# Arcadia-Science/arcadia-microscopy-tools

Hardware: AMD Instinct MI355X
Metric: fields-of-view/sec (4x2048^2 uint16) end-to-end segment+props (higher is better)
Workload: dtype f64; 1 GPU; configs[2]: synthetic 4-channel 2048x2048 uint16 FOVs, DAPI Gaussian+Otsu+open/close+EDT+peak markers+watershed nuclei (SEEDED relief, seeds_first: marker pixels spread first in raster order, cannot tie; SURVEY A.8's plain -EDT relief with exact ties is reported under sublines.a8_exact) + clear_border/relabel + morphology and 4-channel intensity regionprops; mode=weak scaling, 192 FOVs per GPU per step, streams_per_gpu=4, fovs_per_launch=48, max_cells_per_fov=2048, distinct_fovs_per_gpu=8, resident_in_hbm=True

## Files before the change

arcadia_microscopy_tools_amd/_thresholds.py:

```python
from __future__ import annotations

import numpy as np
from scipy import ndimage as ndi


def counts_centers_u16(hist65536: np.ndarray):
    nz = np.flatnonzero(hist65536)
    lo, hi = int(nz[0]), int(nz[-1])
    return hist65536[lo:hi + 1].astype(np.int64), np.arange(lo, hi + 1)


def counts_centers_f64(hist: np.ndarray, vmin: float, vmax: float):
    edges = np.linspace(vmin, vmax, len(hist) + 1)
    return hist.astype(np.int64), (edges[:-1] + edges[1:]) / 2.0


def otsu(counts, bin_centers):
    counts = counts.astype(float)
    if len(bin_centers) == 1:
        return bin_centers[0]
    w_lo = np.cumsum(counts)
    w_hi = np.cumsum(counts[::-1])[::-1]
    weighted = counts * bin_centers
    m_lo = np.cumsum(weighted) / w_lo
# ... 82 lines not shown
        raise RuntimeError("Maximum iteration reached for histogram smoothing")
    k = np.argmin(smooth[maxima[0]:maxima[1] + 1])
    return bin_centers[maxima[0] + k]


def mean_from_hist(counts, values):
    return float(np.sum(counts * values)) / float(np.sum(counts))


def li_from_hist(counts, values, tolerance=None, initial_guess=None, wrap_dtype=None):
    values = values.astype(np.int64)
    counts = np.asarray(counts)
    image_min = int(values[0])
    v = values - image_min
    if wrap_dtype is not None and np.dtype(wrap_dtype).kind == "i" and int(v[-1]) > int(np.iinfo(wrap_dtype).max):
        half = int(np.iinfo(wrap_dtype).max) + 1
        v = (v + half) % (2 * half) - half
        order = np.argsort(v, kind="stable")
        v, counts = v[order], counts[order]
    present = v[counts > 0]
    if present.size == 1:
        return values[0]
    tolerance = tolerance or np.min(np.diff(present)) / 2
    total_sum = np.sum(counts * v)
    total_cnt = np.sum(counts)
    t_next = total_sum / total_cnt if initial_guess is None else initial_guess - image_min
    t_curr = -2 * tolerance
    csum = np.cumsum(counts * v)
    ccnt = np.cumsum(counts)
    with np.errstate(invalid="ignore", divide="ignore"):
        while abs(t_next - t_curr) > tolerance:
            t_curr = t_next
            k = int(np.searchsorted(v, t_curr, side="right")) - 1
            s_le = csum[k] if k >= 0 else 0
            c_le = ccnt[k] if k >= 0 else 0
            mean_back = np.float64(s_le) / np.float64(c_le)
            mean_fore = np.float64(total_sum - s_le) / np.float64(total_cnt - c_le)
            t_next = (mean_back - mean_fore) / (np.log(mean_back) - np.log(mean_fore))
    return t_next + image_min


def prefix_rule(v: np.ndarray, vmin: float, vmax: float, nbins: int = 256):
    v = np.ascontiguousarray(v, dtype=np.float64)
    if (v < 0).any():
        raise ValueError("the prefix order holds for non-negative samples only")
    hi32 = v.view(np.uint64) >> np.uint64(32) << np.uint64(32)
    vlo, vhi = hi32.view(np.float64), (hi32 | np.uint64(0xFFFFFFFF)).view(np.float64)
    edges = np.linspace(vmin, vmax, nbins + 1)
    bins = np.clip(np.searchsorted(edges, vlo, side="right") - 1, 0, nbins - 1)
    centres = (edges[:-1] + edges[1:]) / 2.0
    above = vlo > centres[bins]
    undecided = ((bins < nbins - 1) & (vhi >= edges[bins + 1])) | (~above & (vhi > centres[bins]))
    return bins, above, undecided
```

arcadia_microscopy_tools_amd/csrc/amt_props.hip:

```cpp
#include "amt_internal.h"

#include <vector>

typedef unsigned long long u64;

enum { A_N = 0, A_SY, A_SX, A_SYY, A_SXX, A_SXY, A_C1, A_C2, A_C3, A_NACC };

__global__ void __launch_bounds__(256) rp_init_kernel(u64* __restrict__ acc, int* __restrict__ bbox, size_t nlab) {
    for (size_t i = (size_t)blockIdx.x * 256 + threadIdx.x; i < nlab; i += (size_t)gridDim.x * 256) {
        for (int k = 0; k < A_NACC; ++k) acc[i * A_NACC + k] = 0;
        bbox[i * 4 + 0] = 0x7fffffff;
        bbox[i * 4 + 1] = 0x7fffffff;
        bbox[i * 4 + 2] = -1;
        bbox[i * 4 + 3] = -1;
    }
}

__device__ __forceinline__ u64 sum_sq_upto(u64 m) { return m * (m + 1) * (2 * m + 1) / 6; }

__device__ __forceinline__ double diff_of_products(u64 a, u64 b, u64 c, u64 d) {
    u64 lo1 = a * b, hi1 = __umul64hi(a, b);
    u64 lo2 = c * d, hi2 = __umul64hi(c, d);
    bool neg = (hi1 < hi2) || (hi1 == hi2 && lo1 < lo2);
    u64 hi, lo;
    if (!neg) {
        lo = lo1 - lo2;
        hi = hi1 - hi2 - (lo1 < lo2 ? 1 : 0);
    } else {
        lo = lo2 - lo1;
        hi = hi2 - hi1 - (lo2 < lo1 ? 1 : 0);
    }
    double v = (double)hi * 18446744073709551616.0 + (double)lo;
    return neg ? -v : v;
}

__global__ void __launch_bounds__(256) rp_bbox_kernel(const int* __restrict__ labels, int* __restrict__ bbox, int H,
                                                      int W, int max_label) {
    const int lane = threadIdx.x & 63;
    const int x = blockIdx.x * 64 + lane;
    const int yb = (blockIdx.y * 4 + (threadIdx.x >> 6)) * 8;
    if (yb >= H) return;
    const size_t n = (size_t)H * W;
    const int plane = blockIdx.z;
    int labs[8];
#pragma unroll
    for (int k = 0; k < 8; ++k) {
        const int y = yb + k;
        int v = 0;
        if (x < W && y < H) v = labels[(size_t)plane * n + (size_t)y * W + x];
        labs[k] = (v < 0 || v > max_label) ? 0 : v;
    }
#pragma unroll
    for (int k = 0; k < 8; ++k) {
        const int lab = labs[k];
        const int left = __shfl_up(lab, 1);
        const bool head = (lane == 0) || (left != lab);
        const u64 heads = __ballot(head);
        if (lab != 0 && head) {
            const u64 later = heads & ~((2ull << lane) - 1ull);
            const int end_lane = later ? (__ffsll((long long)later) - 2) : 63;
            int* B = bbox + ((size_t)plane * max_label + (lab - 1)) * 4;
            atomicMin(&B[0], yb + k);
            atomicMin(&B[1], x);
            atomicMax(&B[2], yb + k);
            atomicMax(&B[3], x + (end_lane - lane));
        }
    }
}

__device__ __forceinline__ u64 wave_sum_u64(u64 v) {
#pragma unroll
    for (int off = 32; off >= 1; off >>= 1) v += __shfl_xor(v, off);
    return v;
}
__device__ __forceinline__ unsigned wave_min_u32(unsigned v) {
#pragma unroll
    for (int off = 32; off >= 1; off >>= 1) {
        unsigned t = __shfl_xor(v, off);
        v = t < v ? t : v;
    }
    return v;
}
__device__ __forceinline__ unsigned wave_max_u32(unsigned v) {
#pragma unroll
    for (int off = 32; off >= 1; off >>= 1) {
        unsigned t = __shfl_xor(v, off);
        v = t > v ? t : v;
    }
    return v;
}

constexpr int RP_MAXC = 4;
__global__ void __launch_bounds__(64) rp_label_kernel(const int* __restrict__ labels, const int* __restrict__ bbox,
                                                      const int* __restrict__ hoff, const int* __restrict__ htot,
                                                      int2* __restrict__ rows, size_t cap, u64* __restrict__ acc,
                                                      const uint16_t* __restrict__ inten, int C, int c0, int nc,
                                                      double* __restrict__ itable, int H, int W, int max_label,
                                                      int want_morph) {
    const int plane = blockIdx.y;
    const int l = blockIdx.x;
    const int lane = threadIdx.x;
    const size_t li = (size_t)plane * max_label + l;
    const int y0 = bbox[li * 4 + 0], x0 = bbox[li * 4 + 1], y1 = bbox[li * 4 + 2], x1 = bbox[li * 4 + 3];
    if (y1 < y0) {
        if (itable && lane < 4 * nc) itable[(li * C + c0) * 4 + lane] = 0.0;
        return;
    }
    const size_t n = (size_t)H * W;
    const int* L = labels + (size_t)plane * n;
    const uint16_t* I = inten ? inten + ((size_t)plane * C + c0) * n : nullptr;
    const int want = l + 1;
    const bool rows_ok = want_morph && (size_t)htot[plane] <= cap;
    int2* myrows = rows + (size_t)plane * cap + (size_t)hoff[li];
    u64 cnt = 0, sy = 0, sx = 0, syy = 0, sxx = 0, sxy = 0;
    u64 s[RP_MAXC], q[RP_MAXC];
    unsigned mn[RP_MAXC], mx[RP_MAXC];
#pragma unroll
    for (int c = 0; c < RP_MAXC; ++c) {
        s[c] = 0;
        q[c] = 0;
        mn[c] = 0xffffffffu;
        mx[c] = 0;
    }
    constexpr int RPS = 3;
    for (int yb = y0; yb <= y1; yb += RPS) {
        int rmin[RPS], rmax[RPS];
#pragma unroll
        for (int j = 0; j < RPS; ++j) {
            rmin[j] = 0x7fffffff;
            rmax[j] = -1;
        }
        for (int xb = x0; xb <= x1; xb += 64) {
            const int x = xb + lane;
            unsigned bcnt = 0, bsy = 0;
            const int xc = x <= x1 ? x : x1;
            int lv[RPS];
#pragma unroll
            for (int j = 0; j < RPS; ++j) {
                const int yc = yb + j <= y1 ? yb + j : y1;
                lv[j] = L[(size_t)yc * W + xc];
            }
            unsigned iv[RPS][RP_MAXC];
            if (I) {
#pragma unroll
                for (int j = 0; j < RPS; ++j) {
                    const int yc = yb + j <= y1 ? yb + j : y1;
#pragma unroll
                    for (int c = 0; c < RP_MAXC; ++c) iv[j][c] = I[(size_t)(c < nc ? c : 0) * n + (size_t)yc * W + xc];
                }
            }
#pragma unroll
            for (int j = 0; j < RPS; ++j)
                if (x > x1 || yb + j > y1) lv[j] = 0;
#pragma unroll
            for (int j = 0; j < RPS; ++j) {
                const int y = yb + j;
                const bool m = lv[j] == want;
                if (m) {
                    bcnt += 1u;
                    bsy += (unsigned)y;
                    syy += (u64)(unsigned)y * (unsigned)y;
                    if (I) {
#pragma unroll
                        for (int c = 0; c < RP_MAXC; ++c)
                            if (c < nc) {
                                const unsigned v = iv[j][c];
                                s[c] += v;
                                q[c] += (u64)v * v;
                                mn[c] = v < mn[c] ? v : mn[c];
                                mx[c] = v > mx[c] ? v : mx[c];
                            }
                    }
                }
                const u64 bal = __ballot(m);
                if (bal) {
                    const int first = xb + __ffsll((long long)bal) - 1;
                    const int last = xb + 63 - __clzll((long long)bal);
                    rmin[j] = first < rmin[j] ? first : rmin[j];
                    rmax[j] = last > rmax[j] ? last : rmax[j];
                }
            }
            cnt += bcnt;
            sy += bsy;
            sx += (u64)(unsigned)x * bcnt;
            sxx += (u64)(unsigned)x * (unsigned)x * bcnt;
            sxy += (u64)(unsigned)x * bsy;
        }
        if (rows_ok && lane == 0) {
#pragma unroll
            for (int j = 0; j < RPS; ++j)
                if (yb + j <= y1) myrows[yb + j - y0] = make_int2(rmin[j], rmax[j]);
        }
    }
    cnt = wave_sum_u64(cnt);
    if (want_morph) {
        sy = wave_sum_u64(sy);
        sx = wave_sum_u64(sx);
        syy = wave_sum_u64(syy);
        sxx = wave_sum_u64(sxx);
        sxy = wave_sum_u64(sxy);
        if (lane == 0) {
            u64* A = acc + li * A_NACC;
            A[A_N] = cnt;
            A[A_SY] = sy;
            A[A_SX] = sx;
            A[A_SYY] = syy;
            A[A_SXX] = sxx;
            A[A_SXY] = sxy;
        }
    }
    if (itable) {
#pragma unroll
        for (int c = 0; c < RP_MAXC; ++c)
            if (c < nc) {
                const u64 S = wave_sum_u64(s[c]), Q = wave_sum_u64(q[c]);
                const unsigned lo = wave_min_u32(mn[c]), hi = wave_max_u32(mx[c]);
                if (lane == 0) {
                    double* t = itable + (li * C + c0 + c) * 4;
                    if (cnt == 0) {
                        t[0] = t[1] = t[2] = t[3] = 0.0;
                    } else {
                        const double dn = (double)cnt;
                        t[0] = (double)S / dn;
                        t[1] = (double)hi;
                        t[2] = (double)lo;
                        const double nv = diff_of_products(cnt, Q, S, S);
                        const double var = nv / (dn * dn);
                        t[3] = sqrt(var < 0.0 ? 0.0 : var);
                    }
                }
            }
    }
}

constexpr int PR_ROWS = 64, PR_IN = 60, PR_BATCH = 17, PR_NBATCH = (PR_ROWS + 4) / PR_BATCH;
static_assert(PR_BATCH * PR_NBATCH == PR_ROWS + 4, "row batches must tile the strip");

__global__ void __launch_bounds__(256) rp_perimeter_rows_kernel(const int* __restrict__ labels, u64* __restrict__ acc,
                                                                int H, int W, int max_label, int* __restrict__ bbox) {
    const int lane = threadIdx.x & 63;
    const int strip = blockIdx.x * 4 + (threadIdx.x >> 6);
    if (strip * PR_IN >= W) return;
    const int plane = blockIdx.z;
    const size_t n = (size_t)H * W;
    const int* L = labels + (size_t)plane * n;
    const int x = strip * PR_IN - 2 + lane;
    const int y0 = blockIdx.y * PR_ROWS;
    const bool xin = x >= 0 && x < W;
    const bool inner = xin && lane >= 2 && lane < 2 + PR_IN;
    const unsigned ml = (unsigned)max_label;
    u64* accp = acc + (size_t)plane * max_label * A_NACC;
    int* bbp = bbox ? bbox + (size_t)plane * max_label * 4 : nullptr;

    const int xc = x < 0 ? 0 : (x < W ? x : W - 1);
    auto load_row = [&](int y) -> int {
        const int yc = y < 0 ? 0 : (y < H ? y : H - 1);
        return L[(size_t)yc * W + xc];
    };
    int cur[PR_BATCH], nxt[PR_BATCH];
#pragma unroll
    for (int j = 0; j < PR_BATCH; ++j) cur[j] = load_row(y0 - 2 + j);
    int v1 = 0, v1l = 0, v1r = 0, v2 = 0, v2l = 0, v2r = 0;
    int wA = 0, wAl = 0, wAr = 0, wB = 0, wBl = 0, wBr = 0;
    for (int b = 0; b < PR_NBATCH; ++b) {
        if (b + 1 < PR_NBATCH) {
#pragma unroll
            for (int j = 0; j < PR_BATCH; ++j) nxt[j] = load_row(y0 - 2 + (b + 1) * PR_BATCH + j);
        }
#pragma unroll
        for (int j = 0; j < PR_BATCH; ++j) {
            const int r = y0 - 2 + b * PR_BATCH + j;
            int v0 = cur[j];
            v0 = (xin && r >= 0 && r < H && (unsigned)(v0 - 1) < ml) ? v0 : 0;
            if (__ballot((v0 | v1 | v2 | wB) != 0) == 0ull) continue;
            const int v0l = amt_lane_left(v0), v0r = amt_lane_right(v0);
            const bool b1 = v1 != 0 && (v2 != v1 || v0 != v1 || v1l != v1 || v1r != v1);
            const int w1 = b1 ? (v1 | (int)0x80000000) : v1;
            const int w1l = amt_lane_left(w1), w1r = amt_lane_right(w1);
            const int yb = r - 1;
            if (bbp && yb >= y0 && yb < y0 + PR_ROWS) {
                const bool live = inner && v1 != 0, head = live && v1l != v1;
                const bool q0 = head && v2 != v1, q2 = head && v0 != v1, q1 = head && v2l != v1 && v0l != v1;
                const bool q3 = live && v1r != v1 && v2r != v1 && v0r != v1;
                if (__ballot(q0 || q1 || q2 || q3)) {
                    int* B = bbp + (size_t)(v1 - 1) * 4;
                    if (q0) atomicMin(&B[0], yb);
                    if (q2) atomicMax(&B[2], yb);
                    if (q1) atomicMin(&B[1], x);
                    if (q3) atomicMax(&B[3], x);
                }
            }
            const int yo = r - 2;
            if (inner && wA < 0 && yo >= y0 && yo < y0 + PR_ROWS) {
                const int key = wA;
                const int code = 1 + 2 * ((wB == key) + (w1 == key) + (wAl == key) + (wAr == key)) +
                                 10 * ((wBl == key) + (wBr == key) + (w1l == key) + (w1r == key));
                constexpr unsigned long long M1 = (1ull << 5) | (1ull << 7) | (1ull << 15) | (1ull << 17) | (1ull << 25) | (1ull << 27);
                constexpr unsigned long long M2 = (1ull << 21) | (1ull << 33), M3 = (1ull << 13) | (1ull << 23);
                const int cls = ((M1 >> code) & 1ull) ? A_C1 : ((M2 >> code) & 1ull) ? A_C2 : ((M3 >> code) & 1ull) ? A_C3 : -1;
                if (cls >= 0) atomicAdd(&accp[(size_t)((key & 0x7fffffff) - 1) * A_NACC + cls], 1ull);
            }
            wB = wA, wBl = wAl, wBr = wAr;
            wA = w1, wAl = w1l, wAr = w1r;
            v2 = v1, v2l = v1l, v2r = v1r;
            v1 = v0, v1l = v0l, v1r = v0r;
        }
#pragma unroll
        for (int j = 0; j < PR_BATCH; ++j) cur[j] = nxt[j];
    }
}

__global__ void __launch_bounds__(256) rp_heights_kernel(const int* __restrict__ bbox, int* __restrict__ hoff,
                                                         int max_label) {
    const int plane = blockIdx.y;
    for (int l = blockIdx.x * 256 + threadIdx.x; l < max_label; l += gridDim.x * 256) {
        const int* B = bbox + ((size_t)plane * max_label + l) * 4;
        hoff[(size_t)plane * max_label + l] = B[2] >= B[0] ? B[2] - B[0] + 1 : 0;
    }
}

constexpr int HULL_HMAX = 48, HULL_WMAX = 250;

__device__ __forceinline__ long long floor_div(long long a, long long b) {
    long long q = a / b;
    return (a % b != 0 && a < 0) ? q - 1 : q;
}
__device__ __forceinline__ long long ceil_div(long long a, long long b) {
    long long q = a / b;
    return (a % b != 0 && a > 0) ? q + 1 : q;
}

template <bool CROWS>
__global__ void __launch_bounds__(64) rp_hull_kernel(const int* __restrict__ bbox, const int* __restrict__ hoff,
                                                     const int* __restrict__ htot, const int2* __restrict__ rows,
                                                     int2* __restrict__ chainL, int2* __restrict__ chainR, size_t cap,
                                                     double* __restrict__ table, int max_label, int skip_h,
                                                     int2* __restrict__ crows) {
    const int plane = blockIdx.y;
    const int l = blockIdx.x * 64 + threadIdx.x;
    if (l >= max_label) return;
    const size_t li = (size_t)plane * max_label + l;
    double* trow = CROWS ? nullptr : table + li * AMT_RP_NCOLS;
    const int miny = bbox[li * 4 + 0], maxy = bbox[li * 4 + 2];
    if (maxy < miny) {
        if (!CROWS && skip_h == 0) trow[AMT_RP_AREA_CONVEX] = 0.0;
        return;
    }
    const int h = maxy - miny + 1;
    if (h <= skip_h && bbox[li * 4 + 3] - bbox[li * 4 + 1] + 1 <= HULL_WMAX) return;
    const size_t off = (size_t)hoff[li];
    if ((size_t)htot[plane] > cap || off + (size_t)h > cap) {
        if (!CROWS) trow[AMT_RP_AREA_CONVEX] = __longlong_as_double(0x7ff8000000000000ll);
        return;
    }
    const int2* r = rows + (size_t)plane * cap + off;
    int2* CL = chainL + (size_t)plane * 3 * cap + 3 * off;
    int2* CR = chainR + (size_t)plane * 3 * cap + 3 * off;
    int nl = 0, nr = 0;
    for (int Y = 2 * miny - 1; Y <= 2 * maxy + 1; ++Y) {
        int mn = 0x7fffffff, mx = -0x7fffffff;
        if (Y & 1) {
// ... 208 lines not shown
        const double n2 = dn * dn;
        const double a = Nxx / n2;
        const double c = Nyy / n2;
        const double b = -Nxy / n2;
        const double tr = (a + c) * 0.5;
        const double hd = (a - c) * 0.5;
        const double rad = sqrt(hd * hd + b * b);
        double l1 = tr + rad, l2 = tr - rad;
        l1 = l1 < 0.0 ? 0.0 : l1;
        l2 = l2 < 0.0 ? 0.0 : l2;
        t[AMT_RP_AXIS_MAJOR] = 4.0 * sqrt(l1);
        t[AMT_RP_AXIS_MINOR] = 4.0 * sqrt(l2);
        t[AMT_RP_ECCENTRICITY] = l1 == 0.0 ? 0.0 : sqrt(1.0 - l2 / l1);
        double orient;
        if (Nxx == Nyy) {
            orient = (Nxy > 0.0) ? -0.78539816339744828 : 0.78539816339744828;
        } else {
            orient = 0.5 * atan2(-2.0 * b, c - a);
        }
        t[AMT_RP_ORIENTATION] = orient;
    }
}

__global__ void __launch_bounds__(256) rp_solidity_kernel(double* __restrict__ table, size_t nlab) {
    for (size_t i = (size_t)blockIdx.x * 256 + threadIdx.x; i < nlab; i += (size_t)gridDim.x * 256) {
        double* t = table + i * AMT_RP_NCOLS;
        t[AMT_RP_SOLIDITY] = t[AMT_RP_AREA] > 0.0 ? t[AMT_RP_AREA] / t[AMT_RP_AREA_CONVEX] : 0.0;
    }
}

extern "C" int amt_regionprops(amt_ctx* ctx, const int32_t* labels, const uint16_t* intensity, int C, double* table_dev,
                               double* itable_dev, int nplanes, int H, int W, int max_label) {
    AMT_REQUIRE(labels && (table_dev || itable_dev) && nplanes >= 0 && H > 0 && W > 0 && max_label >= 0,
                "regionprops: bad arguments");
    AMT_REQUIRE(!intensity == !itable_dev && (!itable_dev || C >= 1),
                "regionprops: the intensity planes (C >= 1) and the intensity table go together");
    AMT_TRY(amt_set_device(ctx));
    const bool want_morph = table_dev != nullptr;
    if (nplanes == 0 || max_label == 0) return AMT_OK;
    const size_t n = (size_t)H * W;
    const size_t nlab = (size_t)nplanes * max_label;
    const size_t cap = want_morph ? n : 1;
    amt_scratch s(ctx);
    amt_buf<u64> acc(s, nlab * A_NACC);
    amt_buf<int> bbox(s, nlab * 4);
    amt_buf<int> hoff(s, nlab);
    amt_buf<int> htot(s, nplanes);
    amt_buf<int2> rows(s, (size_t)nplanes * cap);
    amt_buf<int2> chainL(s, (size_t)nplanes * 3 * cap);
    amt_buf<int2> chainR(s, (size_t)nplanes * 3 * cap);
    AMT_TRY(s.commit());
    hipLaunchKernelGGL(rp_init_kernel, dim3(amt_grid_for(nlab, 256, 1024)), dim3(256), 0, ctx->stream, acc, bbox, nlab);
    AMT_LAUNCH_CHECK();
    if (want_morph) {
        const int nstrips = (W + PR_IN - 1) / PR_IN;
        dim3 gper((nstrips + 3) / 4, (H + PR_ROWS - 1) / PR_ROWS, nplanes);
        hipLaunchKernelGGL(rp_perimeter_rows_kernel, gper, dim3(256), 0, ctx->stream, labels, acc, H, W, max_label, bbox);
    } else {
        hipLaunchKernelGGL(rp_bbox_kernel, dim3((W + 63) / 64, (H + 31) / 32, nplanes), dim3(256), 0, ctx->stream,
                           labels, bbox, H, W, max_label);
    }
    AMT_LAUNCH_CHECK();
    hipLaunchKernelGGL(rp_heights_kernel, dim3(amt_grid_for(max_label, 256, 256), nplanes), dim3(256), 0, ctx->stream,
                       bbox, hoff, max_label);
    AMT_LAUNCH_CHECK();
    AMT_TRY(amt_scan_excl(ctx, hoff, max_label, (size_t)max_label, htot, nplanes));
    const int groups = intensity ? (C + RP_MAXC - 1) / RP_MAXC : 1;
    for (int g = 0; g < groups; ++g) {
        const int c0 = g * RP_MAXC;
        const int nc = intensity ? ((C - c0) < RP_MAXC ? (C - c0) : RP_MAXC) : 0;
        hipLaunchKernelGGL(rp_label_kernel, dim3(max_label, nplanes), dim3(64), 0, ctx->stream, labels, bbox, hoff, htot,
                           rows, cap, acc, intensity, C, c0, nc, intensity ? itable_dev : (double*)nullptr, H, W,
                           max_label, (want_morph && g == 0) ? 1 : 0);
        AMT_LAUNCH_CHECK();
    }
    if (want_morph) {
        hipLaunchKernelGGL(rp_final_kernel, dim3(amt_grid_for(nlab, 256, 1024)), dim3(256), 0, ctx->stream, acc, bbox,
                           table_dev, nlab);
        AMT_LAUNCH_CHECK();
        const int skip_h = HULL_HMAX;
        hipLaunchKernelGGL(rp_hull_lds_kernel<false>, dim3((max_label + 31) / 32, nplanes), dim3(64), 0, ctx->stream, bbox,
                           hoff, htot, rows, cap, table_dev, max_label, (int2*)nullptr);
        AMT_LAUNCH_CHECK();
        hipLaunchKernelGGL(rp_hull_kernel<false>, dim3((max_label + 63) / 64, nplanes), dim3(64), 0, ctx->stream, bbox,
                           hoff, htot, rows, chainL, chainR, cap, table_dev, max_label, skip_h, (int2*)nullptr);
        AMT_LAUNCH_CHECK();
        hipLaunchKernelGGL(rp_solidity_kernel, dim3(amt_grid_for(nlab, 256, 1024)), dim3(256), 0, ctx->stream,
                           table_dev, nlab);
        AMT_LAUNCH_CHECK();
    }
    return AMT_OK;
}

__global__ void __launch_bounds__(256) bbox_init_kernel(int* __restrict__ bbox, size_t nlab) {
    for (size_t i = (size_t)blockIdx.x * 256 + threadIdx.x; i < nlab; i += (size_t)gridDim.x * 256) {
        bbox[i * 4 + 0] = 0x7fffffff;
        bbox[i * 4 + 1] = 0x7fffffff;
        bbox[i * 4 + 2] = -1;
        bbox[i * 4 + 3] = -1;
    }
}

__global__ void __launch_bounds__(64) rp_intensity_f64_kernel(const int* __restrict__ labels, const int* __restrict__ bbox,
                                                              const double* __restrict__ inten, int C,
                                                              double* __restrict__ itable, int H, int W, int max_label) {
    const int plane = blockIdx.y, l = blockIdx.x, lane = threadIdx.x;
    const size_t li = (size_t)plane * max_label + l;
    const int y0 = bbox[li * 4 + 0], x0 = bbox[li * 4 + 1], y1 = bbox[li * 4 + 2], x1 = bbox[li * 4 + 3];
    double* out = itable + li * (size_t)C * 4;
    if (y1 < y0) {
        for (int i = lane; i < C * 4; i += 64) out[i] = 0.0;
        return;
    }
    const size_t n = (size_t)H * W;
    const int* lab = labels + (size_t)plane * n;
    auto wsum = [&](double v) {
#pragma unroll
        for (int o = 32; o > 0; o >>= 1) v += __shfl_xor(v, o);
        return v;
    };
    for (int c = 0; c < C; ++c) {
        const double* img = inten + ((size_t)plane * C + c) * n;
        double s = 0.0, cnt = 0.0, mn = __longlong_as_double(0x7ff0000000000000ll), mx = -mn;
        for (int y = y0; y <= y1; ++y)
            for (int x = x0 + lane; x <= x1; x += 64)
                if (lab[(size_t)y * W + x] == l + 1) {
                    const double v = img[(size_t)y * W + x];
                    s += v;
                    cnt += 1.0;
                    mn = v < mn ? v : mn;
                    mx = v > mx ? v : mx;
                }
        s = wsum(s);
        cnt = wsum(cnt);
#pragma unroll
        for (int o = 32; o > 0; o >>= 1) {
            const double a = __shfl_xor(mn, o), b = __shfl_xor(mx, o);
            mn = a < mn ? a : mn;
            mx = b > mx ? b : mx;
        }
        const double mean = s / cnt;
        double q = 0.0;
        for (int y = y0; y <= y1; ++y)
            for (int x = x0 + lane; x <= x1; x += 64)
                if (lab[(size_t)y * W + x] == l + 1) {
                    const double d = img[(size_t)y * W + x] - mean;
                    q += d * d;
                }
        q = wsum(q);
        if (lane == 0) {
            out[c * 4 + 0] = mean;
            out[c * 4 + 1] = mx;
            out[c * 4 + 2] = mn;
            out[c * 4 + 3] = sqrt(q / cnt);
        }
    }
}

extern "C" int amt_regionprops_intensity_f64(amt_ctx* ctx, const int32_t* labels, const double* intensity, int C,
                                             double* table_dev, int nplanes, int H, int W, int max_label) {
    AMT_TRY(amt_set_device(ctx));
    AMT_REQUIRE(labels && intensity && table_dev && nplanes >= 0 && H > 0 && W > 0 && max_label >= 0 && C >= 1,
                "regionprops_intensity_f64: bad arguments");
    if (nplanes == 0 || max_label == 0) return AMT_OK;
    const size_t nlab = (size_t)nplanes * max_label;
    amt_scratch s(ctx);
    amt_buf<int> bbox(s, nlab * 4);
    AMT_TRY(s.commit());
    hipLaunchKernelGGL(bbox_init_kernel, dim3(amt_grid_for(nlab, 256, 1024)), dim3(256), 0, ctx->stream, bbox, nlab);
    AMT_LAUNCH_CHECK();
    hipLaunchKernelGGL(rp_bbox_kernel, dim3((W + 63) / 64, (H + 31) / 32, nplanes), dim3(256), 0, ctx->stream, labels, bbox,
                       H, W, max_label);
    AMT_LAUNCH_CHECK();
    hipLaunchKernelGGL(rp_intensity_f64_kernel, dim3(max_label, nplanes), dim3(64), 0, ctx->stream, labels, bbox, intensity, C,
                       table_dev, H, W, max_label);
    AMT_LAUNCH_CHECK();
    return AMT_OK;
}

extern "C" int amt_label_bboxes(amt_ctx* ctx, const int32_t* labels, int32_t* bbox_dev, int nplanes, int H, int W,
                                int max_label) {
    AMT_TRY(amt_set_device(ctx));
    AMT_REQUIRE(labels && bbox_dev && nplanes >= 0 && H > 0 && W > 0 && max_label >= 1, "label_bboxes: bad arguments");
    if (nplanes == 0) return AMT_OK;
    const size_t nlab = (size_t)nplanes * max_label;
    hipLaunchKernelGGL(bbox_init_kernel, dim3(amt_grid_for(nlab, 256, 1024)), dim3(256), 0, ctx->stream, bbox_dev, nlab);
    AMT_LAUNCH_CHECK();
    hipLaunchKernelGGL(rp_bbox_kernel, dim3((W + 63) / 64, (H + 31) / 32, nplanes), dim3(256), 0, ctx->stream, labels,
                       bbox_dev, H, W, max_label);
    AMT_LAUNCH_CHECK();
    return AMT_OK;
}


__global__ void __launch_bounds__(64) rpx_quad_kernel(const int* __restrict__ labels, const int* __restrict__ bbox,
                                                      double* __restrict__ table, int H, int W, int max_label,
                                                      int want_euler, int want_crofton) {
    __shared__ unsigned hist[16];
    const int plane = blockIdx.y, l = blockIdx.x, lane = threadIdx.x;
    const size_t li = (size_t)plane * max_label + l;
    if (lane < 16) hist[lane] = 0;
    __syncthreads();
    const int y0 = bbox[li * 4 + 0], x0 = bbox[li * 4 + 1], y1 = bbox[li * 4 + 2], x1 = bbox[li * 4 + 3];
    const int* L = labels + (size_t)plane * H * W;
    const int want = l + 1;
    if (y1 >= y0) {
        for (int xb = x0; xb <= x1 + 1; xb += 64) {
            const int x = xb + lane;
            const bool col = x <= x1 + 1;
            unsigned up = 0, upl = 0;
            for (int y = y0; y <= y1 + 1; ++y) {
                unsigned c = 0, cl = 0;
                if (col && y <= y1) {
                    if (x <= x1) c = L[(size_t)y * W + x] == want;
                    if (x - 1 >= x0) cl = L[(size_t)y * W + x - 1] == want;
                }
                const unsigned code = c | (up << 1) | (cl << 2) | (upl << 3);
                if (col && code != 0 && code != 15) atomicAdd(&hist[code], 1u);
                up = c;
                upl = cl;
            }
        }
    }
    __syncthreads();
    if (lane == 0) {
        double* t = table + li * AMT_RPX_NCOLS;
        long long h[16];
        for (int k = 0; k < 16; ++k) h[k] = hist[k];
        if (want_euler) t[AMT_RPX_COL_EULER_NUMBER] = (double)(h[8] - h[6] - h[14]);
        if (want_crofton) {
            const double pi = 3.141592653589793, s2 = sqrt(2.0);
            const double coefs[16] = {0, pi / 4 * (1 + 1 / s2), pi / (4 * s2), pi / (2 * s2), 0, pi / 4 * (1 + 1 / s2),
                                      0, pi / (4 * s2), pi / 4, pi / 2, pi / (4 * s2), pi / (4 * s2), pi / 4, pi / 2, 0, 0};
            double p = 0.0;
            for (int k = 0; k < 16; ++k) p += coefs[k] * (double)h[k];
            t[AMT_RPX_COL_PERIMETER_CROFTON] = y1 >= y0 ? p : 0.0;
        }
    }
}

constexpr int HOLE_SMALL = 64;
__device__ __forceinline__ u64 row_fill(u64 r, u64 b) {
// ... 284 lines not shown
                }
#pragma unroll
        for (int o = 32; o >= 1; o >>= 1) {
            s += __shfl_xor(s, o);
            sy += __shfl_xor(sy, o);
            sx += __shfl_xor(sx, o);
        }
        if (lane == 0) {
            const double ly = (double)sy / (double)s, lx = (double)sx / (double)s;
            out[c * 4 + 0] = ly + (double)y0;
            out[c * 4 + 1] = lx + (double)x0;
            out[c * 4 + 2] = ly;
            out[c * 4 + 3] = lx;
        }
    }
}

extern "C" int amt_regionprops_ext(amt_ctx* ctx, const int32_t* labels, const void* intensity, int in_code, int C,
                                   int columns, double* table_dev, double* wtable_dev, int nplanes, int H, int W,
                                   int max_label) {
    const unsigned cols = (unsigned)columns;
    const bool want_w = (cols & AMT_RPX_CENTROID_WEIGHTED) != 0;
    const bool want_m = (cols & ~AMT_RPX_CENTROID_WEIGHTED) != 0;
    AMT_REQUIRE(labels && nplanes >= 0 && H > 0 && W > 0 && max_label >= 0 && cols != 0 && (cols & ~AMT_RPX_ALL) == 0,
                "regionprops_ext: bad arguments");
    AMT_REQUIRE(!table_dev == !want_m, "regionprops_ext: the morphology table and its column bits go together");
    AMT_REQUIRE(want_w == !!intensity && want_w == !!wtable_dev && (!want_w || C >= 1),
                "regionprops_ext: the intensity planes (C >= 1), the weighted table and AMT_RPX_CENTROID_WEIGHTED go "
                "together");
    AMT_REQUIRE(!want_w || in_code == AMT_U16 || in_code == AMT_F64, "regionprops_ext: intensity must be AMT_U16 or AMT_F64");
    AMT_TRY(amt_set_device(ctx));
    if (nplanes == 0 || max_label == 0) return AMT_OK;
    const bool euler = cols & (AMT_RPX_EULER_NUMBER | AMT_RPX_PERIMETER_CROFTON);
    const bool filled = cols & AMT_RPX_AREA_FILLED, feret = cols & AMT_RPX_FERET_DIAMETER_MAX;
    const bool moments = cols & (AMT_RPX_CENTROID_LOCAL | AMT_RPX_INERTIA_TENSOR | AMT_RPX_INERTIA_EIGVALS);
    const bool scan = filled || feret || moments;
    const size_t n = (size_t)H * W;
    const size_t nlab = (size_t)nplanes * max_label;
    const size_t cap = feret ? n : 1;
    const size_t hwords = filled ? (size_t)H * ((W + 63) / 64) : 0;
    amt_scratch s(ctx);
    amt_buf<u64> acc(s, nlab * A_NACC);
    amt_buf<int> bbox(s, nlab * 4);
    amt_buf<int> hoff(s, nlab);
    amt_buf<int> htot(s, nplanes);
    amt_buf<int2> rows(s, (size_t)nplanes * cap);
    amt_buf<int2> crows(s, (size_t)nplanes * cap);
    amt_buf<int2> chainL(s, (size_t)nplanes * 3 * cap);
    amt_buf<int2> chainR(s, (size_t)nplanes * 3 * cap);
    amt_buf<u64> hscratch(s, (size_t)nplanes * 2 * hwords);
    AMT_TRY(s.commit());
    hipLaunchKernelGGL(rp_init_kernel, dim3(amt_grid_for(nlab, 256, 1024)), dim3(256), 0, ctx->stream, acc, bbox, nlab);
    AMT_LAUNCH_CHECK();
    hipLaunchKernelGGL(rp_bbox_kernel, dim3((W + 63) / 64, (H + 31) / 32, nplanes), dim3(256), 0, ctx->stream, labels,
                       bbox, H, W, max_label);
    AMT_LAUNCH_CHECK();
    if (scan) {
        hipLaunchKernelGGL(rp_heights_kernel, dim3(amt_grid_for(max_label, 256, 256), nplanes), dim3(256), 0, ctx->stream,
                           bbox, hoff, max_label);
        AMT_LAUNCH_CHECK();
        AMT_TRY(amt_scan_excl(ctx, hoff, max_label, (size_t)max_label, htot, nplanes));
        hipLaunchKernelGGL(rp_label_kernel, dim3(max_label, nplanes), dim3(64), 0, ctx->stream, labels, bbox, hoff, htot,
                           rows, cap, acc, (const uint16_t*)nullptr, 1, 0, 0, (double*)nullptr, H, W, max_label, 1);
        AMT_LAUNCH_CHECK();
    }
    if (euler) {
        hipLaunchKernelGGL(rpx_quad_kernel, dim3(max_label, nplanes), dim3(64), 0, ctx->stream, labels, bbox, table_dev, H,
                           W, max_label, (cols & AMT_RPX_EULER_NUMBER) ? 1 : 0, (cols & AMT_RPX_PERIMETER_CROFTON) ? 1 : 0);
        AMT_LAUNCH_CHECK();
    }
    if (filled) {
        hipLaunchKernelGGL(rpx_holes_small_kernel, dim3(max_label, nplanes), dim3(64), 0, ctx->stream, labels, bbox, acc,
                           table_dev, H, W, max_label);
        AMT_LAUNCH_CHECK();
        hipLaunchKernelGGL(rpx_holes_large_kernel, dim3(nplanes), dim3(256), 0, ctx->stream, labels, bbox, acc, table_dev,
                           hscratch, hwords, H, W, max_label);
        AMT_LAUNCH_CHECK();
    }
    if (feret) {
        hipLaunchKernelGGL(rp_hull_lds_kernel<true>, dim3((max_label + 31) / 32, nplanes), dim3(64), 0, ctx->stream, bbox,
                           hoff, htot, rows, cap, (double*)nullptr, max_label, crows);
        AMT_LAUNCH_CHECK();
        hipLaunchKernelGGL(rp_hull_kernel<true>, dim3((max_label + 63) / 64, nplanes), dim3(64), 0, ctx->stream, bbox, hoff,
                           htot, rows, chainL, chainR, cap, (double*)nullptr, max_label, HULL_HMAX, crows);
        AMT_LAUNCH_CHECK();
        hipLaunchKernelGGL(rpx_feret_kernel, dim3(max_label, nplanes), dim3(64), 0, ctx->stream, bbox, hoff, htot, crows,
                           cap, table_dev, max_label);
        AMT_LAUNCH_CHECK();
    }
    if (moments) {
        hipLaunchKernelGGL(rpx_moments_kernel, dim3(amt_grid_for(nlab, 256, 1024)), dim3(256), 0, ctx->stream, acc, bbox,
                           table_dev, nlab, columns);
        AMT_LAUNCH_CHECK();
    }
    if (want_w) {
        if (in_code == AMT_U16)
            hipLaunchKernelGGL((rpx_weighted_kernel<uint16_t, u64>), dim3(max_label, nplanes), dim3(64), 0, ctx->stream,
                               labels, bbox, (const uint16_t*)intensity, C, wtable_dev, H, W, max_label);
        else
            hipLaunchKernelGGL((rpx_weighted_kernel<double, double>), dim3(max_label, nplanes), dim3(64), 0, ctx->stream,
                               labels, bbox, (const double*)intensity, C, wtable_dev, H, W, max_label);
        AMT_LAUNCH_CHECK();
    }
    return AMT_OK;
}


constexpr int COLOC_MAXC = 4, COLOC_MAXP = 6;
struct coloc_launch {
    int chan[COLOC_MAXC];
    int nch;
    int out[COLOC_MAXP];
    int swap[COLOC_MAXP];
};
__host__ __device__ __forceinline__ int coloc_slot_a(int k) { return k < 3 ? 0 : (k < 5 ? 1 : 2); }
__host__ __device__ __forceinline__ int coloc_slot_b(int k) { return k < 3 ? k + 1 : (k < 5 ? k - 1 : 3); }
// ... 202 lines not shown
    for (int off = 32; off > 0; off >>= 1) {
        const double a0 = __shfl_xor(mna, off), a1 = __shfl_xor(mxa, off);
        const double b0 = __shfl_xor(mnb, off), b1 = __shfl_xor(mxb, off);
        mna = a0 < mna ? a0 : mna;
        mxa = a1 > mxa ? a1 : mxa;
        mnb = b0 < mnb ? b0 : mnb;
        mxb = b1 > mxb ? b1 : mxb;
    }
    const double ma = sa / cnt, mb = sb / cnt;
    double cab = 0, caa = 0, cbb = 0;
    for (int y = y0; y <= y1; ++y)
        for (int x = x0 + lane; x <= x1; x += 64)
            if (lab[(size_t)y * W + x] == l + 1) {
                const double da = A[(size_t)y * W + x] - ma, db = B[(size_t)y * W + x] - mb;
                cab += da * db;
                caa += da * da;
                cbb += db * db;
            }
    cab = wsum(cab), caa = wsum(caa), cbb = wsum(cbb);
    if (lane == 0) {
        const double nan = __longlong_as_double(0x7ff8000000000000ll);
        const bool constant = !(mna < mxa) || !(mnb < mxb);
        const double den = sqrt(caa * cbb), oden = sqrt(qa * qb);
        o[AMT_COLOC_PEARSON] = (constant || den == 0.0) ? nan : cab / den;
        o[AMT_COLOC_OVERLAP] = oden == 0.0 ? nan : pab / oden;
        o[AMT_COLOC_M1] = sa != 0.0 ? aif / sa : 0.0;
        o[AMT_COLOC_M2] = sb != 0.0 ? bif / sb : 0.0;
        o[AMT_COLOC_INTERSECTION1] = na != 0.0 ? nab / na : 0.0;
        o[AMT_COLOC_INTERSECTION2] = nb != 0.0 ? nab / nb : 0.0;
    }
}

extern "C" int amt_colocalization(amt_ctx* ctx, const int32_t* labels, const void* intensity, int in_code, int C,
                                  const double* thresholds_dev, const int32_t* pairs_host, int npairs,
                                  double* table_dev, int nplanes, int H, int W, int max_label) {
    AMT_REQUIRE(labels && intensity && thresholds_dev && pairs_host && table_dev && nplanes >= 0 && H > 0 && W > 0 &&
                    max_label >= 0 && C >= 2 && npairs >= 1,
                "colocalization: bad arguments");
    AMT_REQUIRE(in_code == AMT_U16 || in_code == AMT_F64, "colocalization: intensity must be AMT_U16 or AMT_F64");
    AMT_REQUIRE((size_t)H * W <= 0xffffffffull, "colocalization: planes of more than 2^32 - 1 pixels are not supported");
    for (int p = 0; p < npairs; ++p) {
        const int i = pairs_host[2 * p], j = pairs_host[2 * p + 1];
        AMT_REQUIRE(i >= 0 && i < C && j >= 0 && j < C && i != j,
                    "colocalization: pair %d = (%d, %d) must name two different channels below %d", p, i, j, C);
    }
    AMT_TRY(amt_set_device(ctx));
    if (nplanes == 0 || max_label == 0) return AMT_OK;
    const size_t nlab = (size_t)nplanes * max_label;
    amt_scratch s(ctx);
    amt_buf<int> bbox(s, nlab * 4);
    AMT_TRY(s.commit());
    hipLaunchKernelGGL(bbox_init_kernel, dim3(amt_grid_for(nlab, 256, 1024)), dim3(256), 0, ctx->stream, bbox, nlab);
    AMT_LAUNCH_CHECK();
    hipLaunchKernelGGL(rp_bbox_kernel, dim3((W + 63) / 64, (H + 31) / 32, nplanes), dim3(256), 0, ctx->stream, labels, bbox,
                       H, W, max_label);
    AMT_LAUNCH_CHECK();
    if (in_code == AMT_F64) {
        for (int p = 0; p < npairs; ++p) {
            hipLaunchKernelGGL(coloc_f64_kernel, dim3(max_label, nplanes), dim3(64), 0, ctx->stream, labels, bbox,
                               (const double*)intensity, C, thresholds_dev, pairs_host[2 * p], pairs_host[2 * p + 1], p,
                               table_dev, npairs, H, W, max_label);
            AMT_LAUNCH_CHECK();
        }
        return AMT_OK;
    }
    std::vector<char> done((size_t)npairs, 0);
    for (int first = 0; first < npairs; ++first) {
        if (done[first]) continue;
        coloc_launch P;
        P.nch = 0;
        for (int c = 0; c < COLOC_MAXC; ++c) P.chan[c] = 0;
        for (int k = 0; k < COLOC_MAXP; ++k) P.out[k] = -1, P.swap[k] = 0;
        auto slot_of = [&](int ch) {
            for (int c = 0; c < P.nch; ++c)
                if (P.chan[c] == ch) return c;
            return -1;
        };
        for (int p = first; p < npairs; ++p) {
            if (done[p]) continue;
            const int i = pairs_host[2 * p], j = pairs_host[2 * p + 1];
            const int missing = (slot_of(i) < 0 ? 1 : 0) + (slot_of(j) < 0 ? 1 : 0);
            if (P.nch + missing > COLOC_MAXC) continue;
            if (slot_of(i) < 0) P.chan[P.nch++] = i;
            if (slot_of(j) < 0) P.chan[P.nch++] = j;
        }
        for (int p = first; p < npairs; ++p) {
            if (done[p]) continue;
            const int si = slot_of(pairs_host[2 * p]), sj = slot_of(pairs_host[2 * p + 1]);
            if (si < 0 || sj < 0) continue;
            const int a = si < sj ? si : sj, b = si < sj ? sj : si;
            int k = 0;
            while (coloc_slot_a(k) != a || coloc_slot_b(k) != b) ++k;
            if (P.out[k] >= 0) continue;
            P.out[k] = p;
            P.swap[k] = si > sj ? 1 : 0;
            done[p] = 1;
        }
        hipLaunchKernelGGL(coloc_u16_kernel, dim3(max_label, nplanes), dim3(64), 0, ctx->stream, labels, bbox,
                           (const uint16_t*)intensity, C, thresholds_dev, P, table_dev, npairs, H, W, max_label);
        AMT_LAUNCH_CHECK();
    }
    return AMT_OK;
}
```

Before: 15370 FOV/s.

## Move perimeter counting into per-label scan and vectorize bbox kernel

Removes the full-image perimeter-rows kernel, which did per-pixel neighbour classification with global atomics. Perimeter classes are now counted inside the per-label scan kernel using 64-bit ballot masks and bit-sliced adder logic, with a separate strip pass for labels wider than 64 pixels. The bbox kernel becomes a row-streaming version with int4 vector loads, wave-level skipping of empty rows, and atomics only at run heads, tails and vertical edges. The trade is that the per-label kernel does more work, and wide labels are re-read from memory in overlapping strips. A pure-Python reference of the mask rule is also added.

```diff
diff --git a/arcadia_microscopy_tools_amd/_thresholds.py b/arcadia_microscopy_tools_amd/_thresholds.py
--- a/arcadia_microscopy_tools_amd/_thresholds.py
+++ b/arcadia_microscopy_tools_amd/_thresholds.py
@@ -158,3 +158,42 @@
     above = vlo > centres[bins]
     undecided = ((bins < nbins - 1) & (vhi >= edges[bins + 1])) | (~above & (vhi > centres[bins]))
     return bins, above, undecided
+
+
+def perimeter_mask_rule(image: np.ndarray, lanes: int = 64, halo: int = 2):
+    image = np.asarray(image, bool)
+    H, W = image.shape
+    full = (1 << lanes) - 1
+    if W <= lanes:
+        strips = [(0, full)]
+    else:
+        inner = full >> 2 * halo << halo
+        strips = [(xs - halo, inner) for xs in range(0, W, lanes - 2 * halo)]
+    counts = [0, 0, 0]
+    for x_lane0, inner in strips:
+        masks = []
+        for r in range(H):
+            m = 0
+            for lane in range(lanes):
+                x = x_lane0 + lane
+                if 0 <= x < W and image[r, x]:
+                    m |= 1 << lane
+            masks.append(m)
+        masks = [0] + masks + [0]
+        border = [0] + [m & ~(up & dn & (m << 1) & (m >> 1)) & full
+                        for up, m, dn in zip(masks, masks[1:], masks[2:])] + [0]
+        for up, b, dn in zip(border, border[1:], border[2:]):
+            four = [up, dn, b << 1 & full, b >> 1]
+            diag = [up << 1 & full, up >> 1, dn << 1 & full, dn >> 1]
+            for lane in range(lanes):
+                if not (b & inner) >> lane & 1:
+                    continue
+                a = sum(v >> lane & 1 for v in four)
+                d = sum(v >> lane & 1 for v in diag)
+                if a in (2, 3) and d <= 2:
+                    counts[0] += 1
+                elif (a, d) in ((0, 2), (1, 3)):
+                    counts[1] += 1
+                elif a == 1 and d in (1, 2):
+                    counts[2] += 1
+    return tuple(counts)
diff --git a/arcadia_microscopy_tools_amd/csrc/amt_props.hip b/arcadia_microscopy_tools_amd/csrc/amt_props.hip
--- a/arcadia_microscopy_tools_amd/csrc/amt_props.hip
+++ b/arcadia_microscopy_tools_amd/csrc/amt_props.hip
@@ -34,38 +34,115 @@
     return neg ? -v : v;
 }
 
-__global__ void __launch_bounds__(256) rp_bbox_kernel(const int* __restrict__ labels, int* __restrict__ bbox, int H,
-                                                      int W, int max_label) {
+constexpr int BX_ROWS = 30, BX_BATCH = 8, BX_NBATCH = (BX_ROWS + 2) / BX_BATCH;
+static_assert(BX_BATCH * BX_NBATCH == BX_ROWS + 2, "row batches must tile the strip");
+
+template <int V>
+struct bx_row {
+    int v[V];
+};
+
+template <int V>
+__device__ __forceinline__ bx_row<V> bx_load(const int* __restrict__ p) {
+    bx_row<V> r;
+    if constexpr (V == 4) {
+        const int4 q = *reinterpret_cast<const int4*>(p);
+        r.v[0] = q.x, r.v[1] = q.y, r.v[2] = q.z, r.v[3] = q.w;
+    } else {
+        r.v[0] = *p;
+    }
+    return r;
+}
+
+template <int V>
+__global__ void __launch_bounds__(256) rp_bbox_rows_kernel(const int* __restrict__ labels, int* __restrict__ bbox, int H,
+                                                           int W, int max_label) {
     const int lane = threadIdx.x & 63;
-    const int x = blockIdx.x * 64 + lane;
-    const int yb = (blockIdx.y * 4 + (threadIdx.x >> 6)) * 8;
-    if (yb >= H) return;
+    const int strip = blockIdx.x * 4 + (threadIdx.x >> 6);
+    if (strip * 64 * V >= W) return;
+    const int plane = blockIdx.z;
     const size_t n = (size_t)H * W;
-    const int plane = blockIdx.z;
-    int labs[8];
-#pragma unroll
-    for (int k = 0; k < 8; ++k) {
-        const int y = yb + k;
-        int v = 0;
-        if (x < W && y < H) v = labels[(size_t)plane * n + (size_t)y * W + x];
-        labs[k] = (v < 0 || v > max_label) ? 0 : v;
-    }
-#pragma unroll
-    for (int k = 0; k < 8; ++k) {
-        const int lab = labs[k];
-        const int left = __shfl_up(lab, 1);
-        const bool head = (lane == 0) || (left != lab);
-        const u64 heads = __ballot(head);
-        if (lab != 0 && head) {
-            const u64 later = heads & ~((2ull << lane) - 1ull);
-            const int end_lane = later ? (__ffsll((long long)later) - 2) : 63;
-            int* B = bbox + ((size_t)plane * max_label + (lab - 1)) * 4;
-            atomicMin(&B[0], yb + k);
-            atomicMin(&B[1], x);
-            atomicMax(&B[2], yb + k);
-            atomicMax(&B[3], x + (end_lane - lane));
-        }
-    }
+    const int* L = labels + (size_t)plane * n;
+    const int x = strip * 64 * V + lane * V;
+    const int y0 = blockIdx.y * BX_ROWS;
+    const bool xin = x < W;
+    const unsigned ml = (unsigned)max_label;
+    int* bbp = bbox + (size_t)plane * max_label * 4;
+    const int xc = xin ? x : W - V;
+    auto load_row = [&](int y) -> bx_row<V> {
+        const int yc = y < 0 ? 0 : (y < H ? y : H - 1);
+        return bx_load<V>(L + (size_t)yc * W + xc);
+    };
+    bx_row<V> cur[BX_BATCH], nxt[BX_BATCH];
+#pragma unroll
+    for (int j = 0; j < BX_BATCH; ++j) cur[j] = load_row(y0 - 1 + j);
+    int e1[V + 2], e2[V + 2];
+#pragma unroll
+    for (int i = 0; i < V + 2; ++i) e1[i] = e2[i] = 0;
+    for (int b = 0; b < BX_NBATCH; ++b) {
+        if (b + 1 < BX_NBATCH) {
+#pragma unroll
+            for (int j = 0; j < BX_BATCH; ++j) nxt[j] = load_row(y0 - 1 + (b + 1) * BX_BATCH + j);
+        }
+#pragma unroll
+        for (int j = 0; j < BX_BATCH; ++j) {
+            const int r = y0 - 1 + b * BX_BATCH + j;
+            const bool rin = xin && r >= 0 && r < H;
+            int e0[V + 2];
+            bool any = false;
+#pragma unroll
+            for (int i = 0; i < V; ++i) {
+                const int v = cur[j].v[i];
+                e0[i + 1] = (rin && (unsigned)(v - 1) < ml) ? v : 0;
+                any = any || e0[i + 1] != 0 || e1[i + 1] != 0;
+            }
+            if (__ballot(any) == 0ull) {
+#pragma unroll
+                for (int i = 0; i < V + 2; ++i) e2[i] = e1[i], e1[i] = 0;
+                continue;
+            }
+            e0[0] = amt_lane_left(e0[V]);
+            e0[V + 1] = amt_lane_right(e0[1]);
+            const int yb = r - 1;
+            if (yb >= y0 && yb < y0 + BX_ROWS) {
+                bool q0[V], q1[V], q2[V], q3[V], ask = false;
+#pragma unroll
+                for (int i = 0; i < V; ++i) {
+                    const int c = e1[i + 1];
+                    const bool head = c != 0 && e1[i] != c, tail = c != 0 && e1[i + 2] != c;
+                    q0[i] = head && e2[i + 1] != c;
+                    q2[i] = head && e0[i + 1] != c;
+                    q1[i] = head && e2[i] != c && e0[i] != c;
+                    q3[i] = tail && e2[i + 2] != c && e0[i + 2] != c;
+                    ask = ask || q0[i] || q1[i] || q2[i] || q3[i];
+                }
+                if (__ballot(ask)) {
+#pragma unroll
+                    for (int i = 0; i < V; ++i) {
+                        int* B = bbp + (size_t)(e1[i + 1] - 1) * 4;
+                        if (q0[i]) atomicMin(&B[0], yb);
+                        if (q2[i]) atomicMax(&B[2], yb);
+                        if (q1[i]) atomicMin(&B[1], x + i);
+                        if (q3[i]) atomicMax(&B[3], x + i);
+                    }
+                }
+            }
+#pragma unroll
+            for (int i = 0; i < V + 2; ++i) e2[i] = e1[i], e1[i] = e0[i];
+        }
+#pragma unroll
+        for (int j = 0; j < BX_BATCH; ++j) cur[j] = nxt[j];
+    }
+}
+
+static void rp_launch_bbox(amt_ctx* ctx, const int* labels, int* bbox, int nplanes, int H, int W, int max_label) {
+    const bool vec = W % 4 == 0 && ((uintptr_t)labels & 15) == 0;
+    const int nstrips = (W + (vec ? 255 : 63)) / (vec ? 256 : 64);
+    const dim3 grid((nstrips + 3) / 4, (H + BX_ROWS - 1) / BX_ROWS, nplanes);
+    if (vec)
+        hipLaunchKernelGGL(rp_bbox_rows_kernel<4>, grid, dim3(256), 0, ctx->stream, labels, bbox, H, W, max_label);
+    else
+        hipLaunchKernelGGL(rp_bbox_rows_kernel<1>, grid, dim3(256), 0, ctx->stream, labels, bbox, H, W, max_label);
 }
 
 __device__ __forceinline__ u64 wave_sum_u64(u64 v) {
@@ -90,7 +167,43 @@
     return v;
 }
 
+struct rp_perim_window {
+    u64 m1 = 0, m2 = 0;
+    u64 b2 = 0, b3 = 0;
+    unsigned c1 = 0, c2 = 0, c3 = 0;
+    __device__ __forceinline__ void push(u64 m0, u64 inner) {
+        const u64 b1 = m1 & ~(m2 & m0 & (m1 << 1) & (m1 >> 1));
+        const u64 c = b2 & inner;
+        if (c) {
+            const u64 p = b3, q = b1, l = b2 << 1, r = b2 >> 1;
+            const u64 x1 = p ^ q, k1 = p & q, x2 = l ^ r, k2 = l & r;
+            const u64 a0 = x1 ^ x2, k3 = x1 & x2;
+            const u64 a1 = k1 ^ k2 ^ k3, a2 = k1 & k2;
+            const u64 dp = b3 << 1, dq = b3 >> 1, dl = b1 << 1, dr = b1 >> 1;
+            const u64 y1 = dp ^ dq, j1 = dp & dq, y2 = dl ^ dr, j2 = dl & dr;
+            const u64 d0 = y1 ^ y2, j3 = y1 & y2;
+            const u64 d1 = j1 ^ j2 ^ j3, d2 = j1 & j2;
+            const u64 a_is0 = ~(a0 | a1 | a2), a_is1 = a0 & ~a1;
+            const u64 w1 = c & a1 & ~(d2 | (d1 & d0));
+            const u64 w2 = c & ((a_is0 & d1 & ~d0) | (a_is1 & d1 & d0));
+            const u64 w3 = c & a_is1 & (d0 ^ d1);
+            c1 += (unsigned)__popcll(w1);
+            c2 += (unsigned)__popcll(w2);
+            c3 += (unsigned)__popcll(w3);
+        }
+        b3 = b2, b2 = b1, m2 = m1, m1 = m0;
+    }
+    __device__ __forceinline__ void flush(u64 inner) {
+        push(0, inner);
+        push(0, inner);
+        m1 = m2 = b2 = b3 = 0;
+    }
+};
+
 constexpr int RP_MAXC = 4;
+enum { RP_SCAN_MOMENTS = 1, RP_SCAN_PERIMETER = 2 };
+constexpr int RP_PSTRIP = 60;
+constexpr u64 RP_PINNER = 0x3ffffffffffffffcull;
 __global__ void __launch_bounds__(64) rp_label_kernel(const int* __restrict__ labels, const int* __restrict__ bbox,
                                                       const int* __restrict__ hoff, const int* __restrict__ htot,
                                                       int2* __restrict__ rows, size_t cap, u64* __restrict__ acc,
@@ -111,6 +224,8 @@
     const uint16_t* I = inten ? inten + ((size_t)plane * C + c0) * n : nullptr;
     const int want = l + 1;
     const bool rows_ok = want_morph && (size_t)htot[plane] <= cap;
+    const bool perim = (want_morph & RP_SCAN_PERIMETER) != 0, perim_here = perim && x1 - x0 < 64;
+    rp_perim_window pw;
     int2* myrows = rows + (size_t)plane * cap + (size_t)hoff[li];
     u64 cnt = 0, sy = 0, sx = 0, syy = 0, sxx = 0, sxy = 0;
     u64 s[RP_MAXC], q[RP_MAXC];
@@ -173,6 +288,7 @@
                     }
                 }
                 const u64 bal = __ballot(m);
+                if (perim_here) pw.push(bal, ~0ull);
                 if (bal) {
                     const int first = xb + __ffsll((long long)bal) - 1;
                     const int last = xb + 63 - __clzll((long long)bal);
@@ -190,6 +306,26 @@
 #pragma unroll
             for (int j = 0; j < RPS; ++j)
                 if (yb + j <= y1) myrows[yb + j - y0] = make_int2(rmin[j], rmax[j]);
+        }
+    }
+    if (perim_here) {
+        pw.flush(~0ull);
+    } else if (perim) {
+        for (int xs = x0; xs <= x1; xs += RP_PSTRIP) {
+            const int x = xs - 2 + lane;
+            const bool xin = x >= x0 && x <= x1;
+            const int xc = x < x0 ? x0 : (x <= x1 ? x : x1);
+            for (int yb = y0; yb <= y1; yb += RPS) {
+                int lv[RPS];
+#pragma unroll
+                for (int j = 0; j < RPS; ++j) {
+                    const int yc = yb + j <= y1 ? yb + j : y1;
+                    lv[j] = L[(size_t)yc * W + xc];
+                }
+#pragma unroll
+                for (int j = 0; j < RPS; ++j) pw.push(__ballot(xin && yb + j <= y1 && lv[j] == want), RP_PINNER);
+            }
+            pw.flush(RP_PINNER);
         }
     }
     cnt = wave_sum_u64(cnt);
@@ -207,6 +343,11 @@
             A[A_SYY] = syy;
             A[A_SXX] = sxx;
             A[A_SXY] = sxy;
+            if (perim) {
+                A[A_C1] = pw.c1;
+                A[A_C2] = pw.c2;
+                A[A_C3] = pw.c3;
+            }
         }
     }
     if (itable) {
@@ -230,83 +371,6 @@
                     }
                 }
             }
-    }
-}
-
-constexpr int PR_ROWS = 64, PR_IN = 60, PR_BATCH = 17, PR_NBATCH = (PR_ROWS + 4) / PR_BATCH;
-static_assert(PR_BATCH * PR_NBATCH == PR_ROWS + 4, "row batches must tile the strip");
-
-__global__ void __launch_bounds__(256) rp_perimeter_rows_kernel(const int* __restrict__ labels, u64* __restrict__ acc,
-                                                                int H, int W, int max_label, int* __restrict__ bbox) {
-    const int lane = threadIdx.x & 63;
-    const int strip = blockIdx.x * 4 + (threadIdx.x >> 6);
-    if (strip * PR_IN >= W) return;
-    const int plane = blockIdx.z;
-    const size_t n = (size_t)H * W;
-    const int* L = labels + (size_t)plane * n;
-    const int x = strip * PR_IN - 2 + lane;
-    const int y0 = blockIdx.y * PR_ROWS;
-    const bool xin = x >= 0 && x < W;
-    const bool inner = xin && lane >= 2 && lane < 2 + PR_IN;
-    const unsigned ml = (unsigned)max_label;
-    u64* accp = acc + (size_t)plane * max_label * A_NACC;
-    int* bbp = bbox ? bbox + (size_t)plane * max_label * 4 : nullptr;
-
-    const int xc = x < 0 ? 0 : (x < W ? x : W - 1);
-    auto load_row = [&](int y) -> int {
-        const int yc = y < 0 ? 0 : (y < H ? y : H - 1);
-        return L[(size_t)yc * W + xc];
-    };
-    int cur[PR_BATCH], nxt[PR_BATCH];
-#pragma unroll
-    for (int j = 0; j < PR_BATCH; ++j) cur[j] = load_row(y0 - 2 + j);
-    int v1 = 0, v1l = 0, v1r = 0, v2 = 0, v2l = 0, v2r = 0;
-    int wA = 0, wAl = 0, wAr = 0, wB = 0, wBl = 0, wBr = 0;
-    for (int b = 0; b < PR_NBATCH; ++b) {
-        if (b + 1 < PR_NBATCH) {
-#pragma unroll
-            for (int j = 0; j < PR_BATCH; ++j) nxt[j] = load_row(y0 - 2 + (b + 1) * PR_BATCH + j);
-        }
-#pragma unroll
-        for (int j = 0; j < PR_BATCH; ++j) {
-            const int r = y0 - 2 + b * PR_BATCH + j;
-            int v0 = cur[j];
-            v0 = (xin && r >= 0 && r < H && (unsigned)(v0 - 1) < ml) ? v0 : 0;
-            if (__ballot((v0 | v1 | v2 | wB) != 0) == 0ull) continue;
-            const int v0l = amt_lane_left(v0), v0r = amt_lane_right(v0);
-            const bool b1 = v1 != 0 && (v2 != v1 || v0 != v1 || v1l != v1 || v1r != v1);
-            const int w1 = b1 ? (v1 | (int)0x80000000) : v1;
-            const int w1l = amt_lane_left(w1), w1r = amt_lane_right(w1);
-            const int yb = r - 1;
-            if (bbp && yb >= y0 && yb < y0 + PR_ROWS) {
-                const bool live = inner && v1 != 0, head = live && v1l != v1;
-                const bool q0 = head && v2 != v1, q2 = head && v0 != v1, q1 = head && v2l != v1 && v0l != v1;
-                const bool q3 = live && v1r != v1 && v2r != v1 && v0r != v1;
-                if (__ballot(q0 || q1 || q2 || q3)) {
-                    int* B = bbp + (size_t)(v1 - 1) * 4;
-                    if (q0) atomicMin(&B[0], yb);
-                    if (q2) atomicMax(&B[2], yb);
-                    if (q1) atomicMin(&B[1], x);
-                    if (q3) atomicMax(&B[3], x);
-                }
-            }
-            const int yo = r - 2;
-            if (inner && wA < 0 && yo >= y0 && yo < y0 + PR_ROWS) {
-                const int key = wA;
-                const int code = 1 + 2 * ((wB == key) + (w1 == key) + (wAl == key) + (wAr == key)) +
-                                 10 * ((wBl == key) + (wBr == key) + (w1l == key) + (w1r == key));
-                constexpr unsigned long long M1 = (1ull << 5) | (1ull << 7) | (1ull << 15) | (1ull << 17) | (1ull << 25) | (1ull << 27);
-                constexpr unsigned long long M2 = (1ull << 21) | (1ull << 33), M3 = (1ull << 13) | (1ull << 23);
-                const int cls = ((M1 >> code) & 1ull) ? A_C1 : ((M2 >> code) & 1ull) ? A_C2 : ((M3 >> code) & 1ull) ? A_C3 : -1;
-                if (cls >= 0) atomicAdd(&accp[(size_t)((key & 0x7fffffff) - 1) * A_NACC + cls], 1ull);
-            }
-            wB = wA, wBl = wAl, wBr = wAr;
-            wA = w1, wAl = w1l, wAr = w1r;
-            v2 = v1, v2l = v1l, v2r = v1r;
-            v1 = v0, v1l = v0l, v1r = v0r;
-        }
-#pragma unroll
-        for (int j = 0; j < PR_BATCH; ++j) cur[j] = nxt[j];
     }
 }
 
@@ -621,14 +685,7 @@
     AMT_TRY(s.commit());
     hipLaunchKernelGGL(rp_init_kernel, dim3(amt_grid_for(nlab, 256, 1024)), dim3(256), 0, ctx->stream, acc, bbox, nlab);
     AMT_LAUNCH_CHECK();
-    if (want_morph) {
-        const int nstrips = (W + PR_IN - 1) / PR_IN;
-        dim3 gper((nstrips + 3) / 4, (H + PR_ROWS - 1) / PR_ROWS, nplanes);
-        hipLaunchKernelGGL(rp_perimeter_rows_kernel, gper, dim3(256), 0, ctx->stream, labels, acc, H, W, max_label, bbox);
-    } else {
-        hipLaunchKernelGGL(rp_bbox_kernel, dim3((W + 63) / 64, (H + 31) / 32, nplanes), dim3(256), 0, ctx->stream,
-                           labels, bbox, H, W, max_label);
-    }
+    rp_launch_bbox(ctx, labels, bbox, nplanes, H, W, max_label);
     AMT_LAUNCH_CHECK();
     hipLaunchKernelGGL(rp_heights_kernel, dim3(amt_grid_for(max_label, 256, 256), nplanes), dim3(256), 0, ctx->stream,
                        bbox, hoff, max_label);
@@ -640,7 +697,7 @@
         const int nc = intensity ? ((C - c0) < RP_MAXC ? (C - c0) : RP_MAXC) : 0;
         hipLaunchKernelGGL(rp_label_kernel, dim3(max_label, nplanes), dim3(64), 0, ctx->stream, labels, bbox, hoff, htot,
                            rows, cap, acc, intensity, C, c0, nc, intensity ? itable_dev : (double*)nullptr, H, W,
-                           max_label, (want_morph && g == 0) ? 1 : 0);
+                           max_label, (want_morph && g == 0) ? (RP_SCAN_MOMENTS | RP_SCAN_PERIMETER) : 0);
         AMT_LAUNCH_CHECK();
     }
     if (want_morph) {
@@ -738,8 +795,7 @@
     AMT_TRY(s.commit());
     hipLaunchKernelGGL(bbox_init_kernel, dim3(amt_grid_for(nlab, 256, 1024)), dim3(256), 0, ctx->stream, bbox, nlab);
     AMT_LAUNCH_CHECK();
-    hipLaunchKernelGGL(rp_bbox_kernel, dim3((W + 63) / 64, (H + 31) / 32, nplanes), dim3(256), 0, ctx->stream, labels, bbox,
-                       H, W, max_label);
+    rp_launch_bbox(ctx, labels, bbox, nplanes, H, W, max_label);
     AMT_LAUNCH_CHECK();
     hipLaunchKernelGGL(rp_intensity_f64_kernel, dim3(max_label, nplanes), dim3(64), 0, ctx->stream, labels, bbox, intensity, C,
                        table_dev, H, W, max_label);
@@ -755,8 +811,7 @@
     const size_t nlab = (size_t)nplanes * max_label;
     hipLaunchKernelGGL(bbox_init_kernel, dim3(amt_grid_for(nlab, 256, 1024)), dim3(256), 0, ctx->stream, bbox_dev, nlab);
     AMT_LAUNCH_CHECK();
-    hipLaunchKernelGGL(rp_bbox_kernel, dim3((W + 63) / 64, (H + 31) / 32, nplanes), dim3(256), 0, ctx->stream, labels,
-                       bbox_dev, H, W, max_label);
+    rp_launch_bbox(ctx, labels, bbox_dev, nplanes, H, W, max_label);
     AMT_LAUNCH_CHECK();
     return AMT_OK;
 }
@@ -1147,8 +1202,7 @@
     AMT_TRY(s.commit());
     hipLaunchKernelGGL(rp_init_kernel, dim3(amt_grid_for(nlab, 256, 1024)), dim3(256), 0, ctx->stream, acc, bbox, nlab);
     AMT_LAUNCH_CHECK();
-    hipLaunchKernelGGL(rp_bbox_kernel, dim3((W + 63) / 64, (H + 31) / 32, nplanes), dim3(256), 0, ctx->stream, labels,
-                       bbox, H, W, max_label);
+    rp_launch_bbox(ctx, labels, bbox, nplanes, H, W, max_label);
     AMT_LAUNCH_CHECK();
     if (scan) {
         hipLaunchKernelGGL(rp_heights_kernel, dim3(amt_grid_for(max_label, 256, 256), nplanes), dim3(256), 0, ctx->stream,
@@ -1156,7 +1210,8 @@
         AMT_LAUNCH_CHECK();
         AMT_TRY(amt_scan_excl(ctx, hoff, max_label, (size_t)max_label, htot, nplanes));
         hipLaunchKernelGGL(rp_label_kernel, dim3(max_label, nplanes), dim3(64), 0, ctx->stream, labels, bbox, hoff, htot,
-                           rows, cap, acc, (const uint16_t*)nullptr, 1, 0, 0, (double*)nullptr, H, W, max_label, 1);
+                           rows, cap, acc, (const uint16_t*)nullptr, 1, 0, 0, (double*)nullptr, H, W, max_label,
+                           RP_SCAN_MOMENTS);
         AMT_LAUNCH_CHECK();
     }
     if (euler) {
@@ -1465,8 +1520,7 @@
     AMT_TRY(s.commit());
     hipLaunchKernelGGL(bbox_init_kernel, dim3(amt_grid_for(nlab, 256, 1024)), dim3(256), 0, ctx->stream, bbox, nlab);
     AMT_LAUNCH_CHECK();
-    hipLaunchKernelGGL(rp_bbox_kernel, dim3((W + 63) / 64, (H + 31) / 32, nplanes), dim3(256), 0, ctx->stream, labels, bbox,
-                       H, W, max_label);
+    rp_launch_bbox(ctx, labels, bbox, nplanes, H, W, max_label);
     AMT_LAUNCH_CHECK();
     if (in_code == AMT_F64) {
         for (int p = 0; p < npairs; ++p) {
```

Result: no change. 15590 FOV/s (median of 4 runs) (+1.4%).
